# schmidtjonathan/Climate2Weather

Measured on AMD Instinct MI355X. Metric: UNet denoise steps/sec (train fwd+bwd+allreduce+AdamW+EMA windows/s), higher is better.
Workload: dtype bf16; 1 GPU; configs/sda_unet.yml default net, 5 vars x window 13 = 65 ch, 128x128, bf16 training step, 128 windows/GPU/step; global_batch=128, parallelism=dp1, params=72132929

## Files before the change

climate2weather_amd/csrc/conv_igemm.hip:

```cpp
#include <cstdlib>

#include "conv_epilogue.h"
#include "knobs.h"
#include "launch.h"

namespace {

constexpr int BN = 128;
constexpr int WBYTES = BN * 128;
constexpr int NSLOT = 3;
template <int NW> struct GCfg {
    static constexpr int BM = 64 * NW;
    static constexpr int NTHREADS = 128 * NW;
    static constexpr int PBYTES = BM * 128;
    static constexpr int ROWS_PER_ROUND = NTHREADS / 8;
    static constexpr int WROUNDS = BN / ROWS_PER_ROUND;
    static constexpr int ROUND_BYTES = NTHREADS * 16;
};

template <typename T> struct Mma;
template <> struct Mma<bf16_t> {
    __device__ static __forceinline__ void run(const u32x4_t& a, const u32x4_t& b, f32x4_t& c) { c = mfma16<bf16_t>(a, b, c); }
};
template <> struct Mma<f16_t> {
// ... 209 lines not shown
            int ih, iw;
            if (!src_pixel<MODE>(p, oh, ow, tap / 3, tap % 3, ih, iw)) continue;
            const T* xp = (const T*)p.x + (((size_t)b * p.Hin + ih) * p.Win + iw) * p.Cin;
            const T* wp = (const T*)p.w + ((size_t)co * NT + tap) * p.Cin;
            if (co >= p.wrows) continue;
            for (int ci = 0; ci < p.Cin; ++ci) acc = fmaf(Elem<T>::ld(wp + ci), Elem<T>::ld(xp + ci), acc);
        }
        if (p.bias && co < p.wrows) acc += p.bias[co];
        if (p.act == C2W_ACT_SILU) acc = silu_f(acc);
        if (p.act == C2W_ACT_RELU) acc = relu_f(acc);
        const size_t off = (size_t)Q * p.ldy + co;
        if (p.mul) {
            float g = Elem<T>::ld((const T*)p.mul + off);
            acc *= (p.mulmode == C2W_MUL_DSILU) ? dsilu_f(g) : g;
        }
        if (p.res) acc += Elem<T>::ld((const T*)p.res + off);
        if (p.act == C2W_ACT_SILU_PAIR && p.y2) {
            Elem<T>::st((T*)p.y + off, acc);
            const float a_ = Elem<T>::ld((const T*)p.y + off);
            Elem<T>::st((T*)p.y + off, silu_f(a_));
            Elem<T>::st((T*)p.y2 + off, dsilu_f(a_));
            continue;
        }
        if (p.act == C2W_ACT_RELU_PAIR && p.y2) {
            Elem<T>::st((T*)p.y + off, acc);
            const float a_ = Elem<T>::ld((const T*)p.y + off);
            Elem<T>::st((T*)p.y + off, relu_f(a_));
            Elem<T>::st((T*)p.y2 + off, a_ > 0.f ? 1.f : 0.f);
            continue;
        }
        Elem<T>::st((T*)p.y + off, acc);
        if (p.y2) Elem<T>::st((T*)p.y2 + off, silu_f(Elem<T>::ld((const T*)p.y + off)));
    }
}

template <typename T, int MODE, int NW>
int launch_tile(const C2wConvArgs& a, long long npix, int nN, hipStream_t st) {
    typedef GCfg<NW> CF;
    constexpr int ESZ = sizeof(T);
    constexpr int lds_loop = NSLOT * (CF::PBYTES + WBYTES), lds_epi = CF::BM * (BN * ESZ + 16);
    constexpr int lds = lds_loop > lds_epi ? lds_loop : lds_epi;
    if (int rc = c2w_lds_optin<conv_igemm_kernel<T, MODE, NW>>(lds)) return rc;
    const int nM = (int)((npix + CF::BM - 1) / CF::BM);
    conv_igemm_kernel<T, MODE, NW><<<nM * nN, CF::NTHREADS, lds, st>>>(a);
    return (int)hipGetLastError();
}

template <typename T, int MODE>
int launch_mode(const C2wConvArgs& a, int naive, hipStream_t st) {
    const long long npix = (long long)a.B * a.Hout * a.Wout;
    if (naive) {
        long long total = npix * a.Cout;
        int grid = (int)((total + 255) / 256 < 65536 ? (total + 255) / 256 : 65536);
        conv_naive_kernel<T, MODE><<<grid, 256, 0, st>>>(a);
        return (int)hipGetLastError();
    }
    const int nN = (a.Cout + BN - 1) / BN;
    const bool small = ((npix + 255) / 256) * nN < c2w_cu_count();
    return small ? launch_tile<T, MODE, 2>(a, npix, nN, st) : launch_tile<T, MODE, 4>(a, npix, nN, st);
}

template <typename T>
int launch_dtype(const C2wConvArgs& a, int naive, hipStream_t st) {
    switch (a.mode) {
        case C2W_CONV_1X1: return launch_mode<T, C2W_CONV_1X1>(a, naive, st);
        case C2W_CONV_S1: return launch_mode<T, C2W_CONV_S1>(a, naive, st);
        case C2W_CONV_S2: return launch_mode<T, C2W_CONV_S2>(a, naive, st);
        case C2W_CONV_UP: return launch_mode<T, C2W_CONV_UP>(a, naive, st);
        case C2W_CONV_TS2: return launch_mode<T, C2W_CONV_TS2>(a, naive, st);
    }
    return C2W_ERR_BAD_ARG;
}

}

namespace {
C2wKnobs read_knobs() {
    C2wKnobs k;
    k.force_gather = getenv("C2W_FORCE_GATHER") != nullptr;
    k.conv_t3 = getenv("C2W_CONV_T3") ? atoi(getenv("C2W_CONV_T3")) : -1;
    k.conv_s2_patch = getenv("C2W_CONV_S2_PATCH") ? atoi(getenv("C2W_CONV_S2_PATCH")) : 0;
    k.ts2_pairs = !(getenv("C2W_TS2_PAIRS") && atoi(getenv("C2W_TS2_PAIRS")) == 0);
    k.wgrad_atomics = getenv("C2W_WGRAD_ATOMICS") != nullptr;
    k.loss_fusion = getenv("C2W_NO_LOSS_FUSION") == nullptr;
    k.half8 = getenv("C2W_NO_HALF8") == nullptr;
    k.half8_db = !(getenv("C2W_HALF8_DB") && atoi(getenv("C2W_HALF8_DB")) == 0);
    k.attn_valu = getenv("C2W_ATTN_VALU") != nullptr;
    return k;
}
C2wKnobs g_knobs = read_knobs();
}
const C2wKnobs& c2w_knobs() { return g_knobs; }
extern "C" void c2w_knobs_reload(void) { g_knobs = read_knobs(); }

extern "C" int c2w_conv_patch_supported(const C2wConvArgs* a, int dtype) {
    (void)dtype;
    return a != nullptr && c2w_conv_patch_eligible(*a) && !c2w_knobs().force_gather ? 1 : 0;
}

extern "C" int c2w_conv_pool2_supported(const C2wConvArgs* a, int dtype) {
    (void)dtype;
    if (a == nullptr || a->mode != C2W_CONV_S1 || a->res != nullptr || a->mul != nullptr || a->y2 != nullptr || a->act != C2W_ACT_NONE ||
        a->ln_x != nullptr || a->lnf_y != nullptr)
        return 0;
    return c2w_conv_patch_eligible(*a) && !c2w_conv_pair_eligible(*a) && !c2w_knobs().force_gather ? 1 : 0;
}

extern "C" int c2w_conv_lnfwd_supported(const C2wConvArgs* a, int dtype) {
    if (a == nullptr || (dtype != C2W_DTYPE_BF16 && dtype != C2W_DTYPE_F16)) return 0;
    if (a->Cout != 128 || a->ldy != 128 || a->mul != nullptr || a->y2 != nullptr || a->act != C2W_ACT_NONE || a->ln_x != nullptr) return 0;
    return c2w_conv_patch_eligible(*a) && !c2w_knobs().force_gather ? 1 : 0;
}

extern "C" int c2w_conv_lnbwd_supported(const C2wConvArgs* a, int dtype) {
    if (a == nullptr || (dtype != C2W_DTYPE_BF16 && dtype != C2W_DTYPE_F16)) return 0;
    if (a->Cout != 128 || a->ldy != 128 || a->mul != nullptr || a->y2 != nullptr || a->act != C2W_ACT_NONE) return 0;
    return c2w_conv_patch_eligible(*a) && !c2w_knobs().force_gather ? 1 : 0;
}

int c2w_conv_splitk_plan_impl(const C2wConvArgs& a, int dtype, unsigned long long* ws_bytes);
extern "C" int c2w_conv_splitk_plan(const C2wConvArgs* a, int dtype, unsigned long long* ws_bytes) {
    if (a == nullptr) return C2W_ERR_BAD_ARG;
    return c2w_conv_splitk_plan_impl(*a, dtype, ws_bytes);
}

extern "C" int c2w_conv_lnfwd_chain_supported(const C2wConvArgs* a, int dtype) {
    if (!c2w_conv_lnfwd_supported(a, dtype)) return 0;
    return a->mode == C2W_CONV_S1 && c2w_conv_patch3_wanted(*a, dtype) ? 1 : 0;
}

extern "C" int c2w_conv_loss_supported(const C2wConvArgs* a, int dtype) {
    if (a == nullptr || (dtype != C2W_DTYPE_BF16 && dtype != C2W_DTYPE_F16)) return 0;
    if (a->mode != C2W_CONV_S1 || a->wrows > 80 || a->Cout > 128 || a->ldy != 128 || a->res != nullptr || a->mul != nullptr || a->y2 != nullptr ||
        a->act != C2W_ACT_NONE || a->ln_x != nullptr || a->lnf_y != nullptr || (a->flags & C2W_CONV_POOL2) != 0)
        return 0;
    if (a->loss_sum != nullptr && (a->loss_eps == nullptr || a->loss_C <= 0 || a->loss_C != a->wrows || (a->loss_lde & 7) != 0 || a->loss_lde < a->loss_C ||
                                   a->loss_lde > 128))
        return 0;
    const C2wKnobs& k = c2w_knobs();
    return !k.force_gather && k.loss_fusion && c2w_conv_patch_eligible(*a) && c2w_conv_patch3_wanted(*a, dtype) ? 1 : 0;
}

extern "C" long long c2w_conv_det_scratch_bytes(const C2wConvArgs* a, int dtype) {
    if (a == nullptr) return C2W_ERR_BAD_ARG;
    if (a->ln_x != nullptr && a->ln_dm != nullptr) {
        if (!c2w_conv_lnbwd_supported(a, dtype)) return C2W_ERR_UNSUPPORTED;
        return (long long)a->B * (a->Hout >> 3) * (a->Wout >> 4) * 128 * (long long)sizeof(float);
    }
    if (a->loss_sum != nullptr) {
        C2wConvArgs g = *a;
        g.loss_sum = nullptr;
        if (!c2w_conv_loss_supported(&g, dtype)) return C2W_ERR_UNSUPPORTED;
        return (long long)a->B * (a->Hout >> 4) * (a->Wout >> 4) * ((a->Cout + 127) / 128) * (long long)sizeof(float);
    }
    return 0;
}

extern "C" int c2w_conv_wpacked_supported(const C2wConvArgs* a, int dtype) {
    if (a == nullptr || (dtype != C2W_DTYPE_BF16 && dtype != C2W_DTYPE_F16)) return 0;
    return !c2w_knobs().force_gather && c2w_conv_patch_eligible(*a) && c2w_conv_patch3_wanted(*a, dtype) ? 1 : 0;
}

extern "C" int c2w_conv_dispatch(const C2wConvArgs* a, int dtype) {
    if (a == nullptr) return C2W_ERR_BAD_ARG;
    const bool gather = c2w_knobs().force_gather;
    if (!gather && c2w_conv_patch_eligible(*a)) return c2w_conv_patch3_wanted(*a, dtype) ? C2W_KERNEL_PATCH_16X16 : C2W_KERNEL_PATCH_8X16;
    if (!gather && c2w_conv_pair_eligible(*a)) return C2W_KERNEL_PATCH_PAIR;
// ... 47 lines not shown
```

climate2weather_amd/csrc/knobs.h:

```cpp
#pragma once

struct C2wKnobs {
    bool force_gather;
    int conv_t3;
    int conv_s2_patch;
    bool ts2_pairs;
    bool wgrad_atomics;
    bool attn_valu;
    bool loss_fusion;
    bool half8;
    bool half8_db;
};

const C2wKnobs& c2w_knobs();
extern "C" void c2w_knobs_reload(void);
```

climate2weather_amd/csrc/wgrad_patch.hip:

```cpp
#include <algorithm>
#include <cstdint>
#include <cstdlib>
#include <utility>
#include "conv_geom.h"

#include "knobs.h"
#include "launch.h"


namespace {

constexpr int NTHREADS = 512;
constexpr int KPX = 128;
constexpr int ABYTES = KPX * 256;
constexpr int PPITCH = 24;
constexpr int NPIECE = 10 * 3;
constexpr int PBYTES = NPIECE * 1024;
constexpr int NSLOT_A = 3, NSLOT_P = 2;
constexpr int PBASE = NSLOT_A * ABYTES;
constexpr int LDS_BYTES = PBASE + NSLOT_P * PBYTES;

struct WpArgs {
    const void* dy;
    const void* x;
    float* dw;
    float* db;
    int B, H, W, Cin, Cout, ldy;
    int up;
    int ktiles, ktiles_per_split;
    float* ws;
    int direct;
    float* wsb;
    int det;
};

struct WpItem {
    const void* dy;
    const void* x;
    float* dw;
    float* db;
};
constexpr int WP_MAX_ITEMS = 16;
struct WpGroupArgs {
    WpArgs c;
    int n;
    int live_per_item;
    unsigned long long ws_item_floats;
    unsigned long long wsb_item_floats;
    WpItem item[WP_MAX_ITEMS];
};



__device__ __forceinline__ uint32_t sel_oob(bool ok, uint32_t v) {
    asm volatile("" : "+v"(v));
    return ok ? v : C2W_OOB;
}

__device__ __forceinline__ uint32_t swzA(int row) { return (uint32_t)(((row & 3) << 2) | ((row >> 2) & 3)); }
__device__ __forceinline__ uint32_t swzP(int pix) { return (uint32_t)((((pix >> 1) & 1) << 1) | (((pix >> 3) & 1) << 2)); }

__device__ __forceinline__ int wp_xcd_order(int bid, int nblk) {
    const int xcd = bid & 7, q = nblk >> 3, r = nblk & 7;
    return (xcd < r ? xcd * (q + 1) : r * (q + 1) + (xcd - r) * q) + (bid >> 3);
}

template <typename T, bool PAIR = false, bool NARROW = false>
__device__ __forceinline__ void wgrad_patch_body(const WpArgs& p, const int L) {
    constexpr int ESZ = sizeof(T);
    constexpr bool BF = ESZ == 2;
    constexpr int COT = 256 / ESZ;
    constexpr int CIB = 128 / ESZ;
    constexpr int MTW = BF ? 4 : 1;
    extern __shared__ __attribute__((aligned(16))) char smem[];

    const int tid = threadIdx.x, lane = tid & 63;
    const int wid = __builtin_amdgcn_readfirstlane(tid >> 6);
    const int li = lane & 15, lg = lane >> 4;
    static_assert(!NARROW || (BF && !PAIR), "narrow-M form: 16-bit, 16-pixel-wide tiles");
    const int mt0 = BF ? (NARROW ? (wid >> 2) * 4 : (wid & 1) * 4) : (wid >> 1);
    const int nt = BF ? (NARROW ? (wid & 3) : (wid >> 1)) : (wid & 1);
    const bool light = NARROW && wid >= 4;

    const int ncib = p.Cin / CIB;
    const int tilesM = (p.Cout + COT - 1) / COT;
    const int tilesMN = tilesM * ncib;
    const int split = L / tilesMN, mn = L - split * tilesMN;
    const int tm = mn / ncib, cb = mn - tm * ncib;
    const int co0 = tm * COT, ci0 = cb * CIB;
    const int H = p.H, W = p.W;
    const int tw = PAIR ? 1 : W >> 4, tpi = (H >> 3) * tw;
    const int t0 = split * p.ktiles_per_split;
    const int t1 = (t0 + p.ktiles_per_split < p.ktiles) ? t0 + p.ktiles_per_split : p.ktiles;

    const int Ws = p.up ? W >> 1 : W;
    const size_t ximg = (size_t)(p.up ? (H >> 1) * Ws : H * W) * p.Cin * ESZ;
    const size_t yimg = (size_t)H * W * p.ldy * ESZ;
    const uint32_t a_step = PAIR ? (uint32_t)(16 * p.ldy * ESZ) : (uint32_t)(2 * W * p.ldy * ESZ);
    auto dy_voff0 = [&](int tid_) -> uint32_t {
        const int row = tid_ >> 4, pc = tid_ & 15;
        const uint32_t lc = (uint32_t)pc ^ swzA(row);
        const int c = co0 + (int)lc * (16 / ESZ);
        if constexpr (PAIR) {
            return sel_oob(c < p.Cout, (uint32_t)((((row >> 4) * 8 + (row & 7)) * p.ldy + c) * ESZ) + (uint32_t)((row >> 3) & 1) * (uint32_t)yimg);
        } else {
            return sel_oob(c < p.Cout, (uint32_t)((((row >> 4) * W + (row & 15)) * p.ldy + c) * ESZ));
        }
    };
    auto patch_piece = [&](int r) -> int {
        const int pc = r * 8 + wid;
        return pc < NPIECE ? pc : NPIECE - 1;
    };
    auto patch_voff = [&](int r, int lane_, int oh0, int ow0) -> uint32_t {
        const int pc = patch_piece(r);
        const int pr = pc / 3, pg = pc - pr * 3;
        const int px = pg * 8 + (lane_ >> 3);
        const uint32_t lanepart = (uint32_t)(((lane_ & 7) ^ swzP(pr * PPITCH + px)) << 4) + (uint32_t)ci0 * ESZ;
        if constexpr (PAIR) {
            const int pimg = px >= 10 ? 1 : 0;
            const int ih = pr - 1, iw = px - 1 - 10 * pimg;
            const bool ok = (unsigned)ih < 8u && (unsigned)iw < 8u && px < 20;
            return sel_oob(ok, (uint32_t)((ih * 8 + iw) * p.Cin) * ESZ + (uint32_t)pimg * (uint32_t)(64 * p.Cin * ESZ) + lanepart);
        } else {
            const int ih = oh0 - 1 + pr, iw = ow0 - 1 + px;
            const bool ok = (unsigned)ih < (unsigned)H && (unsigned)iw < (unsigned)W && px < 18;
            const int spix = p.up ? (ih >> 1) * Ws + (iw >> 1) : ih * W + iw;
            return sel_oob(ok, (uint32_t)(spix * p.Cin) * ESZ + lanepart);
        }
    };

    auto tile_origin = [&](int t, int& b, int& oh0, int& ow0) {
        b = PAIR ? 2 * t : t / tpi;
        const int tt = PAIR ? 0 : t - (t / tpi) * tpi;
        const int ty = tt / tw, tx = tt - ty * tw;
        b = __builtin_amdgcn_readfirstlane(b);
        oh0 = __builtin_amdgcn_readfirstlane(ty << 3);
        ow0 = __builtin_amdgcn_readfirstlane(tx << 4);
    };
    struct TileSrc {
        __amdgpu_buffer_rsrc_t rsrc;
        int oh0, ow0;
        uint32_t aso;
        char* base;
    };
    auto srcA = [&](int t, int sa) {
        int b, oh0, ow0;
        tile_origin(t, b, oh0, ow0);
        const uint32_t nimg = PAIR && b + 1 < p.B ? 2u : 1u;
        TileSrc s;
        s.rsrc = make_rsrc((const char*)p.dy + (size_t)b * yimg, (uint32_t)yimg * nimg);
        s.oh0 = oh0;
        s.ow0 = ow0;
        s.aso = (uint32_t)((oh0 * W + ow0) * p.ldy) * ESZ;
        s.base = smem + sa * ABYTES + wid * 1024;
        return s;
    };
    auto srcP = [&](int t, int sp) {
        int b, oh0, ow0;
        tile_origin(t, b, oh0, ow0);
        const uint32_t nimg = PAIR && b + 1 < p.B ? 2u : 1u;
        TileSrc s;
        s.rsrc = make_rsrc((const char*)p.x + (size_t)b * ximg, (uint32_t)ximg * nimg);
        s.oh0 = oh0;
        s.ow0 = ow0;
        s.aso = 0;
        s.base = smem + PBASE + sp * PBYTES;
        return s;
    };
    auto pieceA = [&](const TileSrc& s, int i, bool live = true) {
        int tid_ = tid;
        asm volatile("" : "+v"(tid_));
        const uint32_t v = dy_voff0(tid_);
        glds16(s.rsrc, s.base + i * 8192, sel_oob(live, v), s.aso + (uint32_t)i * a_step);
    };
    auto pieceP = [&](const TileSrc& s, int r, bool live = true) {
        int lane_ = lane;
        asm volatile("" : "+v"(lane_));
        const uint32_t v = patch_voff(r, lane_, s.oh0, s.ow0);
        glds16(s.rsrc, s.base + patch_piece(r) * 1024, sel_oob(live, v), 0);
    };
    auto issueA = [&](int t, int sa) {
        const TileSrc s = srcA(t, sa);
#pragma unroll
        for (int i = 0; i < 4; ++i) pieceA(s, i);
    };
    auto issueP = [&](int t, int sp) {
        const TileSrc s = srcP(t, sp);
#pragma unroll
        for (int r = 0; r < 4; ++r) pieceP(s, r);
    };

    f32x4_t acc[9][MTW];
#pragma unroll
    for (int t = 0; t < 9; ++t)
#pragma unroll
        for (int m = 0; m < MTW; ++m) acc[t][m] = (f32x4_t){0.f, 0.f, 0.f, 0.f};
    const bool do_bias = p.db != nullptr && cb == 0 && nt == 0;
    f32x4_t accb[MTW];
#pragma unroll
    for (int m = 0; m < MTW; ++m) accb[m] = (f32x4_t){0.f, 0.f, 0.f, 0.f};

    uint32_t offA[MTW][2], offB[9][2];
    if constexpr (BF) {
        const int qq = li >> 2, pp = li & 3;
#pragma unroll
        for (int h = 0; h < 2; ++h) {
            const int row = 8 * lg + qq + 4 * h;
            const uint32_t f = swzA(row);
#pragma unroll
            for (int m = 0; m < MTW; ++m)
                offA[m][h] = (uint32_t)(row * 256 + (((((mt0 + m) * 2 + (pp >> 1)) ^ f) & 15) << 4) + 8 * (pp & 1));
            const int r = lg >> 1, c = 8 * (lg & 1) + qq + 4 * h;
#pragma unroll
            for (int t = 0; t < 9; ++t) {
                const int pix = (r + t / 3) * PPITCH + c + t % 3 + (PAIR ? 2 * (lg & 1) : 0);
                offB[t][h] = (uint32_t)(pix * 128 + (((uint32_t)(nt * 2 + (pp >> 1)) ^ swzP(pix)) << 4) + 8 * (pp & 1));
            }
        }
    }

    if (t0 < t1) {
        issueP(t0, 0);
        issueA(t0, 0);
        const TileSrc s1 = srcA(t0 + 1 < t1 ? t0 + 1 : t0, 1);
#pragma unroll
        for (int i = 0; i < 4; ++i) pieceA(s1, i, t0 + 1 < t1);
    }
    int sa = 0, sp = 0;
    for (int t = t0; t < t1; ++t) {
        asm volatile("s_waitcnt vmcnt(4)" ::: "memory");
        __builtin_amdgcn_s_barrier();
        const bool hasP = t + 1 < t1, hasA = t + 2 < t1;
        const TileSrc nP = srcP(hasP ? t + 1 : t, sp ^ 1), nA = srcA(hasA ? t + 2 : t, sa == 0 ? 2 : sa - 1);
        if constexpr (!BF) {
#pragma unroll
            for (int r = 0; r < 4; ++r) pieceP(nP, r, hasP);
#pragma unroll
            for (int i = 0; i < 4; ++i) pieceA(nA, i, hasA);
        }
        const char* const SA = smem + sa * ABYTES;
        const char* const SP = smem + PBASE + sp * PBYTES;
        if constexpr (BF) {
            const uint32_t sA = (uint32_t)(uintptr_t)SA, sP = (uint32_t)(uintptr_t)SP;
            auto rd = [&](tr_frag& f, uint32_t base, uint32_t o0, uint32_t o1, auto IMMc) {
                constexpr int IMM = decltype(IMMc)::value;
                asm volatile("ds_read_b64_tr_b16 %0, %1 offset:%2" : "=v"(f.lo) : "v"(base + o0), "n"(IMM));
                asm volatile("ds_read_b64_tr_b16 %0, %1 offset:%2" : "=v"(f.hi) : "v"(base + o1), "n"(IMM));
            };
            static_for<4>([&](auto KSc) {
                constexpr int ks = decltype(KSc)::value;
                {
                    const bool first = wid < 4;
                    if ((ks == 0 && first) || (ks == 1 && !first)) {
#pragma unroll
                        for (int r = 0; r < 4; ++r) pieceP(nP, r, hasP);
                    }
                    if ((ks == 2 && first) || (ks == 3 && !first)) {
#pragma unroll
                        for (int i = 0; i < 4; ++i) pieceA(nA, i, hasA);
                    }
                }
                constexpr int PF = 2;
                tr_frag a[MTW], bq[PF + 1];
                rd(a[0], sA, offA[0][0], offA[0][1], IC<ks * 32 * 256>{});
                if (!light) {
#pragma unroll
                    for (int m = 1; m < MTW; ++m) rd(a[m], sA, offA[m][0], offA[m][1], IC<ks * 32 * 256>{});
                }
                static_for<PF>([&](auto Jc) {
                    constexpr int j = decltype(Jc)::value;
                    rd(bq[j], sP, offB[j][0], offB[j][1], IC<ks * 2 * PPITCH * 128>{});
                });
                static_for<9>([&](auto TPc) {
                    constexpr int tp = decltype(TPc)::value;
                    if constexpr (tp + PF < 9) rd(bq[(tp + PF) % (PF + 1)], sP, offB[tp + PF][0], offB[tp + PF][1], IC<ks * 2 * PPITCH * 128>{});
                    constexpr int AHEAD = (tp + PF < 9 ? PF : 8 - tp) * 2;
                    if constexpr (AHEAD == 4) asm volatile("s_waitcnt lgkmcnt(4)" ::: "memory");
                    else if constexpr (AHEAD == 2) asm volatile("s_waitcnt lgkmcnt(2)" ::: "memory");
                    else asm volatile("s_waitcnt lgkmcnt(0)" ::: "memory");
                    __builtin_amdgcn_sched_barrier(0);
                    const bf16x8_t bfr = bq[tp % (PF + 1)].vec();
                    acc[tp][0] = mfma16s<T>(a[0].vec(), bfr, acc[tp][0]);
                    if (!light) {
#pragma unroll
                        for (int m = 1; m < MTW; ++m) acc[tp][m] = mfma16s<T>(a[m].vec(), bfr, acc[tp][m]);
                    }
                    if (tp == 8 && do_bias) {
                        const bf16x8_t ones = __builtin_bit_cast(bf16x8_t, ones16<T>());
                        accb[0] = mfma16s<T>(a[0].vec(), ones, accb[0]);
                        if (!light) {
#pragma unroll
                            for (int m = 1; m < MTW; ++m) accb[m] = mfma16s<T>(a[m].vec(), ones, accb[m]);
                        }
                    }
                    __builtin_amdgcn_sched_barrier(0);
                });
            });
        } else {
#pragma unroll 4
            for (int kk = 0; kk < 32; ++kk) {
                const int row = kk * 4 + lg;
                const float a = *(const float*)(SA + row * 256 + ((((uint32_t)(mt0 * 4 + (li >> 2))) ^ swzA(row)) << 4) + (li & 3) * 4);
                const int r = kk >> 2, c = 4 * (kk & 3) + lg;
#pragma unroll
                for (int tp = 0; tp < 9; ++tp) {
                    const int pix = (r + tp / 3) * PPITCH + c + tp % 3 + (PAIR && (kk & 2) ? 2 : 0);
                    const float bv = *(const float*)(SP + pix * 128 + ((((uint32_t)(nt * 4 + (li >> 2))) ^ swzP(pix)) << 4) + (li & 3) * 4);
                    acc[tp][0] = __builtin_amdgcn_mfma_f32_16x16x4f32(a, bv, acc[tp][0], 0, 0, 0);
                }
                if (do_bias) accb[0] = __builtin_amdgcn_mfma_f32_16x16x4f32(a, 1.0f, accb[0], 0, 0, 0);
            }
        }
        sa = sa == 2 ? 0 : sa + 1;
        sp ^= 1;
    }

    if (t0 >= t1) return;
    if (do_bias && li == 0) {
#pragma unroll
        for (int m = 0; m < MTW; ++m)
#pragma unroll
            for (int r = 0; r < 4; ++r) {
                const int row = (mt0 + m) * 16 + lg * 4 + r;
                const int co = co0 + row;
                if (p.det) {
                    if (p.wsb != nullptr) p.wsb[((size_t)split * tilesM + tm) * COT + row] = accb[m][r];
                    else if (co < p.Cout) p.db[co] = p.db[co] + accb[m][r];
                } else if (co < p.Cout) {
                    atomicAdd(p.db + co, accb[m][r]);
                }
            }
    }
    constexpr int OS = CIB + 4;
    float* const O = (float*)smem;
#pragma unroll
    for (int tp = 0; tp < 9; ++tp) {
        __syncthreads();
#pragma unroll
        for (int m = 0; m < MTW; ++m)
#pragma unroll
            for (int r = 0; r < 4; ++r) O[((mt0 + m) * 16 + lg * 4 + r) * OS + nt * 16 + li] = acc[tp][m][r];
        __syncthreads();
        if (p.ws != nullptr) {
            float* const dst = p.ws + (((size_t)split * tilesMN + mn) * 9 + tp) * (COT * CIB);
            for (int idx = tid; idx < COT * CIB; idx += NTHREADS) dst[idx] = O[(idx / CIB) * OS + (idx % CIB)];
        } else if (p.direct) {
            for (int idx = tid; idx < COT * CIB; idx += NTHREADS) {
                const int row = idx / CIB, col = idx - row * CIB;
                const int co = co0 + row;
                if (co < p.Cout) {
                    float* const d = p.dw + ((size_t)co * 9 + tp) * p.Cin + ci0 + col;
                    *d = *d + O[row * OS + col];
                }
            }
        } else {
            for (int idx = tid; idx < COT * CIB; idx += NTHREADS) {
                const int row = idx / CIB, col = idx - row * CIB;
                const int co = co0 + row;
                if (co < p.Cout) atomicAdd(p.dw + ((size_t)co * 9 + tp) * p.Cin + ci0 + col, O[row * OS + col]);
            }
        }
    }
}

template <typename T, bool PAIR = false, bool NARROW = false>
__global__ __launch_bounds__(NTHREADS, 2) void wgrad_patch_kernel(const WpArgs p) {
    wgrad_patch_body<T, PAIR, NARROW>(p, wp_xcd_order((int)blockIdx.x, (int)gridDim.x));
}

typedef __attribute__((address_space(4))) const char wp_kernarg_t;
__device__ __forceinline__ WpItem wp_item(int it) {
    const WpItem __attribute__((address_space(4)))* tab =
        (const WpItem __attribute__((address_space(4)))*)((wp_kernarg_t*)__builtin_amdgcn_kernarg_segment_ptr() + offsetof(WpGroupArgs, item));
    WpItem r;
    r.dy = tab[it].dy;
    r.x = tab[it].x;
    r.dw = tab[it].dw;
    r.db = tab[it].db;
    return r;
}

template <typename T, bool PAIR = false>
__global__ __launch_bounds__(NTHREADS, 2) void wgrad_patch_group_kernel(const WpGroupArgs g) {
    const int Lg = wp_xcd_order((int)blockIdx.x, (int)gridDim.x);
    const int it = __builtin_amdgcn_readfirstlane(Lg / g.live_per_item);
    const int L = Lg - it * g.live_per_item;
    const WpItem e = wp_item(it);
    WpArgs p = g.c;
    p.dy = e.dy;
    p.x = e.x;
    p.dw = e.dw;
    p.db = e.db;
    p.ws = g.c.ws != nullptr ? g.c.ws + (size_t)it * g.ws_item_floats : nullptr;
    p.wsb = g.c.wsb != nullptr ? g.c.wsb + (size_t)it * g.wsb_item_floats : nullptr;
    wgrad_patch_body<T, PAIR, false>(p, L);
}

struct WgradBiasReduce {
    const float* wsb;
    float* db;
    int cols, tpo, nmain;
};
static inline WgradBiasReduce bias_reduce_of(const float* wsb, float* db, int cols, int nsplit, int nmain) {
    WgradBiasReduce br;
    br.wsb = wsb; br.db = db; br.cols = cols; br.tpo = det_reduce_tpo(nsplit); br.nmain = nmain;
    return br;
}

#ifndef C2W_RED_COLS
#define C2W_RED_COLS 64
#endif
template <int COT, int CIB>
__device__ __forceinline__ void wgrad_reduce_body(const float* __restrict__ ws, float* __restrict__ dw, int nsplit, int tilesMN, int ncib,
                                                  int Cin, int Cout, int nblk) {
    constexpr int RC = C2W_RED_COLS, RG = 256 / RC;
    __shared__ f32x4_t red[RG][RC];
    const size_t per4 = (size_t)tilesMN * 9 * COT * CIB / 4;
    const f32x4_t* ws4 = (const f32x4_t*)ws;
    const int q = threadIdx.x % RC, grp = threadIdx.x / RC;
    for (size_t base = (size_t)blockIdx.x * RC; base < per4; base += (size_t)nblk * RC) {
        const size_t i4 = base + q;
        f32x4_t acc = {0.f, 0.f, 0.f, 0.f};
        if (i4 < per4) {
#pragma unroll 8
            for (int sidx = grp; sidx < nsplit; sidx += RG) acc += ws4[(size_t)sidx * per4 + i4];
        }
        red[grp][q] = acc;
        __syncthreads();
        if (grp == 0 && i4 < per4) {
#pragma unroll
            for (int g2 = 1; g2 < RG; ++g2) acc += red[g2][q];
            const size_t i = i4 * 4;
            const int col = (int)(i % CIB);
            size_t r = i / CIB;
            const int row = (int)(r % COT);
            r /= COT;
            const int tp = (int)(r % 9);
            const int mn = (int)(r / 9);
            const int tm = mn / ncib, cb = mn - tm * ncib;
            const int co = tm * COT + row;
            if (co < Cout) {
                f32x4_t* d = (f32x4_t*)(dw + ((size_t)co * 9 + tp) * Cin + cb * CIB + col);
                *d = *d + acc;
            }
        }
        __syncthreads();
    }
}

template <int COT, int CIB>
__global__ __launch_bounds__(256) void wgrad_reduce_kernel(const float* __restrict__ ws, float* __restrict__ dw, int nsplit, int tilesMN, int ncib,
                                                           int Cin, int Cout, WgradBiasReduce br) {
    if ((int)blockIdx.x >= br.nmain) {
        det_reduce_body(br.wsb, br.db, nsplit, Cout, Cout, 0, br.tpo, br.cols, (int)blockIdx.x - br.nmain);
        return;
    }
    wgrad_reduce_body<COT, CIB>(ws, dw, nsplit, tilesMN, ncib, Cin, Cout, br.nmain);
}
template <int COT, int CIB>
__global__ __launch_bounds__(256) void wgrad_reduce_group_kernel(const WpGroupArgs g, int nsplit, int tilesMN, int ncib, WgradBiasReduce br) {
    const int it = (int)blockIdx.y;
    const WpItem e = wp_item(it);
    if ((int)blockIdx.x >= br.nmain) {
        if (e.db != nullptr)
            det_reduce_body(g.c.wsb + (size_t)it * g.wsb_item_floats, e.db, nsplit, g.c.Cout, g.c.Cout, 0, br.tpo, br.cols, (int)blockIdx.x - br.nmain);
        return;
    }
    wgrad_reduce_body<COT, CIB>(g.c.ws + (size_t)it * g.ws_item_floats, e.dw, nsplit, tilesMN, ncib, g.c.Cin, g.c.Cout, br.nmain);
}

template <int ESZ, bool PAIR>
static void split_plan(const C2wConvArgs& a, int& ktiles, int& tilesMN, int& nsplit, int& ktiles_per_split) {
    constexpr int COT = 256 / ESZ, CIB = 128 / ESZ;
    ktiles = PAIR ? ((a.B + 1) >> 1) * (a.Hout >> 3) : a.B * (a.Hout >> 3) * (a.Wout >> 4);
    tilesMN = ((a.Cout + COT - 1) / COT) * (a.Cin / CIB);
    nsplit = c2w_cu_count() / tilesMN;
    if (nsplit > ktiles) nsplit = ktiles;
    if (nsplit < 1) nsplit = 1;
    ktiles_per_split = (ktiles + nsplit - 1) / nsplit;
    nsplit = (ktiles + ktiles_per_split - 1) / ktiles_per_split;
}

template <int ESZ, bool PAIR>
static size_t ws_need(const C2wConvArgs& a) {
    constexpr int COT = 256 / ESZ, CIB = 128 / ESZ;
    int ktiles, tilesMN, nsplit, per;
    split_plan<ESZ, PAIR>(a, ktiles, tilesMN, nsplit, per);
    const size_t bias_rows = (a.flags & C2W_CONV_DETERMINISTIC) ? (size_t)nsplit * ((a.Cout + COT - 1) / COT) * COT * sizeof(float) : 0;
    return nsplit > 1 ? (size_t)nsplit * tilesMN * 9 * COT * CIB * sizeof(float) + bias_rows : 0;
}

template <typename T, bool PAIR, bool NARROW = false>
int launch(const C2wConvArgs& a, float* dw, float* db, float* ws, size_t ws_bytes, hipStream_t st) {
    constexpr int ESZ = sizeof(T);
    constexpr int COT = 256 / ESZ, CIB = 128 / ESZ;
    WpArgs p;
    p.dy = a.y; p.x = a.x; p.dw = dw; p.db = db;
    p.B = a.B; p.H = a.Hout; p.W = a.Wout; p.Cin = a.Cin; p.Cout = a.Cout; p.ldy = a.ldy;
    p.up = a.mode == C2W_CONV_UP ? 1 : 0;
    int tilesMN, nsplit;
    split_plan<ESZ, PAIR>(a, p.ktiles, tilesMN, nsplit, p.ktiles_per_split);
    if (int rc = c2w_lds_optin<wgrad_patch_kernel<T, PAIR, NARROW>>(LDS_BYTES)) return rc;
    const size_t need = (size_t)nsplit * tilesMN * 9 * COT * CIB * sizeof(float);
    const int bias_cols = (tilesMN / (a.Cin / CIB)) * COT;
    p.det = (a.flags & C2W_CONV_DETERMINISTIC) ? 1 : 0;
    if (p.det) {
        if (c2w_knobs().wgrad_atomics) return C2W_ERR_BAD_ARG;
        if (nsplit > 1 && (ws == nullptr || need + (size_t)nsplit * bias_cols * sizeof(float) > ws_bytes)) return C2W_ERR_BAD_ARG;
    }
    p.ws = (ws != nullptr && need <= ws_bytes && nsplit > 1 && !c2w_knobs().wgrad_atomics) ? ws : nullptr;
    p.wsb = p.det && nsplit > 1 && db != nullptr ? ws + need / sizeof(float) : nullptr;
    p.direct = nsplit == 1 && !c2w_knobs().wgrad_atomics ? 1 : 0;
    wgrad_patch_kernel<T, PAIR, NARROW><<<tilesMN * nsplit, NTHREADS, LDS_BYTES, st>>>(p);
    if (p.ws != nullptr) {
        const size_t per_split = (size_t)tilesMN * 9 * COT * CIB;
        const int grid = (int)std::min<size_t>((per_split / 4 + C2W_RED_COLS - 1) / C2W_RED_COLS, 8192);
        const int extra = p.wsb != nullptr ? det_reduce_blocks(nsplit, a.Cout) : 0;
        wgrad_reduce_kernel<COT, CIB><<<grid + extra, 256, 0, st>>>(p.ws, dw, nsplit, tilesMN, a.Cin / CIB, a.Cin, a.Cout,
                                                                    bias_reduce_of(p.wsb, db, bias_cols, nsplit, grid));
    }
    return (int)hipGetLastError();
}

static void group_plan(int n, int tilesMN, int ktiles, int& nsplit, int& ktiles_per_split) {
    const int T = n * tilesMN, cus = c2w_cu_count();
    double best = 1e30;
    nsplit = 1;
    for (int r = 0; r <= 4; ++r) {
        int ns = r == 0 ? 1 : (cus * r) / T;
        if (ns < 1) ns = 1;
        if (ns > ktiles) ns = ktiles;
        const int per = (ktiles + ns - 1) / ns;
        ns = (ktiles + per - 1) / per;
        const int rounds = (T * ns + cus - 1) / cus;
        const double cost = rounds * (per * 4.1 + (ns > 1 ? 28.0 : 16.0)) + (ns > 1 ? 10.0 : 0.0);
        if (cost < best - 1e-9) {
            best = cost;
            nsplit = ns;
        }
    }
    ktiles_per_split = (ktiles + nsplit - 1) / nsplit;
}

template <int ESZ, bool PAIR>
static size_t group_ws_need(const C2wConvArgs& a, int n) {
    constexpr int COT = 256 / ESZ, CIB = 128 / ESZ;
    int ktiles, tilesMN, ns1, per1, nsplit, per;
    split_plan<ESZ, PAIR>(a, ktiles, tilesMN, ns1, per1);
    group_plan(n, tilesMN, ktiles, nsplit, per);
    const size_t bias_rows = (a.flags & C2W_CONV_DETERMINISTIC) ? (size_t)n * nsplit * ((a.Cout + COT - 1) / COT) * COT * sizeof(float) : 0;
    return nsplit > 1 ? (size_t)n * nsplit * tilesMN * 9 * COT * CIB * sizeof(float) + bias_rows : 0;
}

template <typename T, bool PAIR>
int launch_group(const C2wConvArgs& a, const C2wWgradItem* items, int n, float* ws, size_t ws_bytes, hipStream_t st) {
    constexpr int ESZ = sizeof(T);
    constexpr int COT = 256 / ESZ, CIB = 128 / ESZ;
    WpGroupArgs g;
    WpArgs& p = g.c;
    p.dy = nullptr; p.x = nullptr; p.dw = nullptr; p.db = nullptr;
    p.B = a.B; p.H = a.Hout; p.W = a.Wout; p.Cin = a.Cin; p.Cout = a.Cout; p.ldy = a.ldy;
    p.up = a.mode == C2W_CONV_UP ? 1 : 0;
    int tilesMN, ns1, per1, nsplit;
    split_plan<ESZ, PAIR>(a, p.ktiles, tilesMN, ns1, per1);
    group_plan(n, tilesMN, p.ktiles, nsplit, p.ktiles_per_split);
    const size_t item_floats = (size_t)nsplit * tilesMN * 9 * COT * CIB;
    const int bias_cols = (tilesMN / (a.Cin / CIB)) * COT;
    p.det = (a.flags & C2W_CONV_DETERMINISTIC) ? 1 : 0;
    const size_t bias_item_floats = p.det ? (size_t)nsplit * bias_cols : 0;
    if (nsplit > 1 && (ws == nullptr || (size_t)n * (item_floats + bias_item_floats) * sizeof(float) > ws_bytes)) return C2W_ERR_BAD_ARG;
    p.ws = nsplit > 1 ? ws : nullptr;
    p.wsb = p.det && nsplit > 1 ? ws + (size_t)n * item_floats : nullptr;
    g.wsb_item_floats = bias_item_floats;
    p.direct = nsplit == 1 ? 1 : 0;
    g.n = n;
    g.live_per_item = tilesMN * nsplit;
    g.ws_item_floats = item_floats;
    for (int i = 0; i < WP_MAX_ITEMS; ++i) {
        const C2wWgradItem& e = items[i < n ? i : n - 1];
        g.item[i].dy = e.dy; g.item[i].x = e.x; g.item[i].dw = e.dw; g.item[i].db = e.dbias;
    }
    if (int rc = c2w_lds_optin<wgrad_patch_group_kernel<T, PAIR>>(LDS_BYTES)) return rc;
    wgrad_patch_group_kernel<T, PAIR><<<g.live_per_item * n, NTHREADS, LDS_BYTES, st>>>(g);
    if (p.ws != nullptr) {
        const size_t per_split = (size_t)tilesMN * 9 * COT * CIB;
        const int grid = (int)std::min<size_t>((per_split / 4 + C2W_RED_COLS - 1) / C2W_RED_COLS, 8192);
        const int extra = p.wsb != nullptr ? det_reduce_blocks(nsplit, a.Cout) : 0;
        wgrad_reduce_group_kernel<COT, CIB><<<dim3(grid + extra, n), 256, 0, st>>>(g, nsplit, tilesMN, a.Cin / CIB,
                                                                                   bias_reduce_of(p.wsb, nullptr, bias_cols, nsplit, grid));
    }
    return (int)hipGetLastError();
}

}

bool c2w_wgrad_patch_group_eligible(const C2wConvArgs& a, int n, int dtype) {
    const bool narrow = dtype != C2W_DTYPE_F32 && !c2w_wgrad_patch_pair(a) && a.Cout <= 80;
    return c2w_wgrad_patch_eligible(a) && n >= 2 && n <= WP_MAX_ITEMS && !narrow && !c2w_knobs().wgrad_atomics;
}

int c2w_wgrad_patch_group(const C2wConvArgs& a, const C2wWgradItem* items, int n, float* ws, size_t ws_bytes, int dtype, hipStream_t st) {
    if (c2w_wgrad_patch_pair(a)) return c2w_by_dtype(dtype, [&](auto t) { return launch_group<decltype(t), true>(a, items, n, ws, ws_bytes, st); });
    return c2w_by_dtype(dtype, [&](auto t) { return launch_group<decltype(t), false>(a, items, n, ws, ws_bytes, st); });
}

size_t c2w_wgrad_patch_group_ws_bytes(const C2wConvArgs& a, int n, int dtype) {
    const bool pair = c2w_wgrad_patch_pair(a);
    if (dtype == C2W_DTYPE_F32) return pair ? group_ws_need<4, true>(a, n) : group_ws_need<4, false>(a, n);
    return pair ? group_ws_need<2, true>(a, n) : group_ws_need<2, false>(a, n);
}

bool c2w_wgrad_patch_pair(const C2wConvArgs& a) {
    return a.mode == C2W_CONV_S1 && a.Win == 8 && a.Hin == 8;
}

bool c2w_wgrad_patch_eligible(const C2wConvArgs& a) {
    if (a.mode == C2W_CONV_UP)
        return a.Hout == 2 * a.Hin && a.Wout == 2 * a.Win && (a.Hout & 7) == 0 && (a.Wout & 15) == 0;
    return a.mode == C2W_CONV_S1 && a.Hin == a.Hout && a.Win == a.Wout && (a.Hin & 7) == 0 && ((a.Win & 15) == 0 || c2w_wgrad_patch_pair(a));
}

int c2w_wgrad_patch(const C2wConvArgs& a, float* dw, float* db, float* ws, size_t ws_bytes, int dtype, hipStream_t st) {
    if (c2w_wgrad_patch_pair(a)) return c2w_by_dtype(dtype, [&](auto t) { return launch<decltype(t), true>(a, dw, db, ws, ws_bytes, st); });
    if (dtype != C2W_DTYPE_F32 && a.Cout <= 80)
        return c2w_by_dtype16(dtype, [&](auto t) { return launch<decltype(t), false, true>(a, dw, db, ws, ws_bytes, st); });
    return c2w_by_dtype(dtype, [&](auto t) { return launch<decltype(t), false>(a, dw, db, ws, ws_bytes, st); });
}

size_t c2w_wgrad_patch_ws_bytes(const C2wConvArgs& a, int dtype) {
    const bool pair = c2w_wgrad_patch_pair(a);
    if (dtype == C2W_DTYPE_F32) return pair ? ws_need<4, true>(a) : ws_need<4, false>(a);
    return pair ? ws_need<2, true>(a) : ws_need<2, false>(a);
}
```

Before: 2781 windows/s.

## Compute upsample-conv weight grads on source grid with folded 2x2 taps

Adds a source-grid variant of the patch-based weight-gradient kernel for nearest-upsample convolutions. Each output-row parity class is handled by its own split. The 3x3 taps collapse onto a 2x2 footprint of the low-resolution input, so each k-step issues 4 MFMA fragments instead of 9, and the results are folded back into 9 taps in the epilogue. This removes redundant multiplies on duplicated upsampled pixels. In exchange it doubles the number of workspace splits and the reduction traffic, and adds index-mapping complexity. It is enabled by default for bf16/fp16 upsample layers with Cout > 80 when the workspace is large enough.

Measured after the change: 2805 windows/s (median of 6 runs). No clear change (+0.9%).

```diff
diff --git a/climate2weather_amd/csrc/conv_igemm.hip b/climate2weather_amd/csrc/conv_igemm.hip
--- a/climate2weather_amd/csrc/conv_igemm.hip
+++ b/climate2weather_amd/csrc/conv_igemm.hip
@@ -315,7 +315,8 @@
     k.conv_s2_patch = getenv("C2W_CONV_S2_PATCH") ? atoi(getenv("C2W_CONV_S2_PATCH")) : 0;
     k.ts2_pairs = !(getenv("C2W_TS2_PAIRS") && atoi(getenv("C2W_TS2_PAIRS")) == 0);
     k.wgrad_atomics = getenv("C2W_WGRAD_ATOMICS") != nullptr;
-    k.loss_fusion = getenv("C2W_NO_LOSS_FUSION") == nullptr;
+    k.wgrad_up_source = !(getenv("C2W_WGRAD_UP_SOURCE") && atoi(getenv("C2W_WGRAD_UP_SOURCE")) == 0);
+    k.loss_fusion =getenv("C2W_NO_LOSS_FUSION") == nullptr;
     k.half8 = getenv("C2W_NO_HALF8") == nullptr;
     k.half8_db = !(getenv("C2W_HALF8_DB") && atoi(getenv("C2W_HALF8_DB")) == 0);
     k.attn_valu = getenv("C2W_ATTN_VALU") != nullptr;
diff --git a/climate2weather_amd/csrc/knobs.h b/climate2weather_amd/csrc/knobs.h
--- a/climate2weather_amd/csrc/knobs.h
+++ b/climate2weather_amd/csrc/knobs.h
@@ -6,6 +6,7 @@
     int conv_s2_patch;
     bool ts2_pairs;
     bool wgrad_atomics;
+    bool wgrad_up_source;
     bool attn_valu;
     bool loss_fusion;
     bool half8;
diff --git a/climate2weather_amd/csrc/wgrad_patch.hip b/climate2weather_amd/csrc/wgrad_patch.hip
--- a/climate2weather_amd/csrc/wgrad_patch.hip
+++ b/climate2weather_amd/csrc/wgrad_patch.hip
@@ -6,6 +6,7 @@
 
 #include "knobs.h"
 #include "launch.h"
+#include "wgrad_upsrc_maps.h"
 
 
 namespace {
@@ -65,7 +66,7 @@
     return (xcd < r ? xcd * (q + 1) : r * (q + 1) + (xcd - r) * q) + (bid >> 3);
 }
 
-template <typename T, bool PAIR = false, bool NARROW = false>
+template <typename T, bool PAIR = false, bool NARROW = false, bool UPSRC = false>
 __device__ __forceinline__ void wgrad_patch_body(const WpArgs& p, const int L) {
     constexpr int ESZ = sizeof(T);
     constexpr bool BF = ESZ == 2;
@@ -78,6 +79,8 @@
     const int wid = __builtin_amdgcn_readfirstlane(tid >> 6);
     const int li = lane & 15, lg = lane >> 4;
     static_assert(!NARROW || (BF && !PAIR), "narrow-M form: 16-bit, 16-pixel-wide tiles");
+    static_assert(!UPSRC || (BF && !PAIR && !NARROW), "source-grid form: 16-bit, 16-pixel-wide tiles, full co tiles");
+    constexpr int NFRAG = UPSRC ? 4 : 9;
     const int mt0 = BF ? (NARROW ? (wid >> 2) * 4 : (wid & 1) * 4) : (wid >> 1);
     const int nt = BF ? (NARROW ? (wid & 3) : (wid >> 1)) : (wid & 1);
     const bool light = NARROW && wid >= 4;
@@ -89,19 +92,22 @@
     const int tm = mn / ncib, cb = mn - tm * ncib;
     const int co0 = tm * COT, ci0 = cb * CIB;
     const int H = p.H, W = p.W;
-    const int tw = PAIR ? 1 : W >> 4, tpi = (H >> 3) * tw;
-    const int t0 = split * p.ktiles_per_split;
+    const int tw = PAIR ? 1 : W >> 4, tpi = (H >> (UPSRC ? 4 : 3)) * tw;
+    const int cls = UPSRC ? upsrc::cls_of(split) : 0;
+    const int t0 = (UPSRC ? upsrc::ksplit_of(split) : split) * p.ktiles_per_split;
     const int t1 = (t0 + p.ktiles_per_split < p.ktiles) ? t0 + p.ktiles_per_split : p.ktiles;
 
     const int Ws = p.up ? W >> 1 : W;
     const size_t ximg = (size_t)(p.up ? (H >> 1) * Ws : H * W) * p.Cin * ESZ;
     const size_t yimg = (size_t)H * W * p.ldy * ESZ;
-    const uint32_t a_step = PAIR ? (uint32_t)(16 * p.ldy * ESZ) : (uint32_t)(2 * W * p.ldy * ESZ);
+    const uint32_t a_step = PAIR ? (uint32_t)(16 * p.ldy * ESZ) : (uint32_t)((UPSRC ? 4 : 2) * W * p.ldy * ESZ);
     auto dy_voff0 = [&](int tid_) -> uint32_t {
         const int row = tid_ >> 4, pc = tid_ & 15;
-        const uint32_t lc = (uint32_t)pc ^ swzA(row);
+        const uint32_t lc = (uint32_t)pc ^ (UPSRC ? upsrc::swz_dy(row) : swzA(row));
         const int c = co0 + (int)lc * (16 / ESZ);
-        if constexpr (PAIR) {
+        if constexpr (UPSRC) {
+            return sel_oob(c < p.Cout, (uint32_t)((((row >> 4) * 2 * W + (row & 15)) * p.ldy + c) * ESZ));
+        } else if constexpr (PAIR) {
             return sel_oob(c < p.Cout, (uint32_t)((((row >> 4) * 8 + (row & 7)) * p.ldy + c) * ESZ) + (uint32_t)((row >> 3) & 1) * (uint32_t)yimg);
         } else {
             return sel_oob(c < p.Cout, (uint32_t)((((row >> 4) * W + (row & 15)) * p.ldy + c) * ESZ));
@@ -109,10 +115,18 @@
     };
     auto patch_piece = [&](int r) -> int {
         const int pc = r * 8 + wid;
-        return pc < NPIECE ? pc : NPIECE - 1;
+        constexpr int NP = UPSRC ? upsrc::NPIECE : NPIECE;
+        return pc < NP ? pc : NP - 1;
     };
     auto patch_voff = [&](int r, int lane_, int oh0, int ow0) -> uint32_t {
         const int pc = patch_piece(r);
+        if constexpr (UPSRC) {
+            const int pr = pc >> 1, px = (pc & 1) * 8 + (lane_ >> 3);
+            const uint32_t lanepart = (uint32_t)(((lane_ & 7) ^ upsrc::swz_patch(pr * upsrc::PITCH + px)) << 4) + (uint32_t)ci0 * ESZ;
+            const int ih = upsrc::patch_ih(oh0, cls, pr), iw = upsrc::patch_iw(ow0, px);
+            const bool ok = (unsigned)ih < (unsigned)(H >> 1) && (unsigned)iw < (unsigned)Ws && px < upsrc::COLS;
+            return sel_oob(ok, (uint32_t)((ih * Ws + iw) * p.Cin) * ESZ + lanepart);
+        }
         const int pr = pc / 3, pg = pc - pr * 3;
         const int px = pg * 8 + (lane_ >> 3);
         const uint32_t lanepart = (uint32_t)(((lane_ & 7) ^ swzP(pr * PPITCH + px)) << 4) + (uint32_t)ci0 * ESZ;
@@ -134,7 +148,7 @@
         const int tt = PAIR ? 0 : t - (t / tpi) * tpi;
         const int ty = tt / tw, tx = tt - ty * tw;
         b = __builtin_amdgcn_readfirstlane(b);
-        oh0 = __builtin_amdgcn_readfirstlane(ty << 3);
+        oh0 = __builtin_amdgcn_readfirstlane(ty << (UPSRC ? 4 : 3));
         ow0 = __builtin_amdgcn_readfirstlane(tx << 4);
     };
     struct TileSrc {
@@ -151,7 +165,7 @@
         s.rsrc = make_rsrc((const char*)p.dy + (size_t)b * yimg, (uint32_t)yimg * nimg);
         s.oh0 = oh0;
         s.ow0 = ow0;
-        s.aso = (uint32_t)((oh0 * W + ow0) * p.ldy) * ESZ;
+        s.aso = (uint32_t)(((oh0 + cls) * W + ow0) * p.ldy) * ESZ;
         s.base = smem + sa * ABYTES + wid * 1024;
         return s;
     };
@@ -205,16 +219,21 @@
         const int qq = li >> 2, pp = li & 3;
 #pragma unroll
         for (int h = 0; h < 2; ++h) {
-            const int row = 8 * lg + qq + 4 * h;
-            const uint32_t f = swzA(row);
+            const int row = UPSRC ? 16 * lg + 8 * h + 2 * qq : 8 * lg + qq + 4 * h;
+            const uint32_t f = UPSRC ? upsrc::swz_dy(row) : swzA(row);
 #pragma unroll
             for (int m = 0; m < MTW; ++m)
                 offA[m][h] = (uint32_t)(row * 256 + (((((mt0 + m) * 2 + (pp >> 1)) ^ f) & 15) << 4) + 8 * (pp & 1));
             const int r = lg >> 1, c = 8 * (lg & 1) + qq + 4 * h;
 #pragma unroll
             for (int t = 0; t < 9; ++t) {
-                const int pix = (r + t / 3) * PPITCH + c + t % 3 + (PAIR ? 2 * (lg & 1) : 0);
-                offB[t][h] = (uint32_t)(pix * 128 + (((uint32_t)(nt * 2 + (pp >> 1)) ^ swzP(pix)) << 4) + 8 * (pp & 1));
+                if constexpr (UPSRC) {
+                    const int pix = (lg + t / 3) * upsrc::PITCH + 4 * h + qq + t % 3;
+                    offB[t][h] = (uint32_t)(pix * 128 + (((uint32_t)(nt * 2 + (pp >> 1)) ^ upsrc::swz_patch(pix)) << 4) + 8 * (pp & 1));
+                } else {
+                    const int pix = (r + t / 3) * PPITCH + c + t % 3 + (PAIR ? 2 * (lg & 1) : 0);
+                    offB[t][h] = (uint32_t)(pix * 128 + (((uint32_t)(nt * 2 + (pp >> 1)) ^ swzP(pix)) << 4) + 8 * (pp & 1));
+                }
             }
         }
     }
@@ -262,30 +281,40 @@
                 }
                 constexpr int PF = 2;
                 tr_frag a[MTW], bq[PF + 1];
-                rd(a[0], sA, offA[0][0], offA[0][1], IC<ks * 32 * 256>{});
+                constexpr int IMMA = UPSRC ? (ks >> 1) * 64 * 256 + (ks & 1) * 256 : ks * 32 * 256;
+                constexpr int IMMB = UPSRC ? (ks >> 1) * 4 * upsrc::PITCH * 128 : ks * 2 * PPITCH * 128;
+                auto bsel = [](auto FRc) {
+                    constexpr int fr = decltype(FRc)::value;
+                    return IC<UPSRC ? 3 * (fr >> 1) + (ks & 1) + (fr & 1) : fr>{};
+                };
+                rd(a[0], sA, offA[0][0], offA[0][1], IC<IMMA>{});
                 if (!light) {
 #pragma unroll
-                    for (int m = 1; m < MTW; ++m) rd(a[m], sA, offA[m][0], offA[m][1], IC<ks * 32 * 256>{});
+                    for (int m = 1; m < MTW; ++m) rd(a[m], sA, offA[m][0], offA[m][1], IC<IMMA>{});
                 }
                 static_for<PF>([&](auto Jc) {
-                    constexpr int j = decltype(Jc)::value;
-                    rd(bq[j], sP, offB[j][0], offB[j][1], IC<ks * 2 * PPITCH * 128>{});
+                    constexpr int j = decltype(bsel(Jc))::value;
+                    rd(bq[decltype(Jc)::value], sP, offB[j][0], offB[j][1], IC<IMMB>{});
                 });
-                static_for<9>([&](auto TPc) {
-                    constexpr int tp = decltype(TPc)::value;
-                    if constexpr (tp + PF < 9) rd(bq[(tp + PF) % (PF + 1)], sP, offB[tp + PF][0], offB[tp + PF][1], IC<ks * 2 * PPITCH * 128>{});
-                    constexpr int AHEAD = (tp + PF < 9 ? PF : 8 - tp) * 2;
+                static_for<NFRAG>([&](auto TPc) {
+                    constexpr int fr = decltype(TPc)::value;
+                    constexpr int tp = UPSRC ? upsrc::g_index(fr >> 1, ks & 1, fr & 1) : fr;
+                    if constexpr (fr + PF < NFRAG) {
+                        constexpr int j = decltype(bsel(IC<fr + PF>{}))::value;
+                        rd(bq[(fr + PF) % (PF + 1)], sP, offB[j][0], offB[j][1], IC<IMMB>{});
+                    }
+                    constexpr int AHEAD = (fr + PF < NFRAG ? PF : NFRAG - 1 - fr) * 2;
                     if constexpr (AHEAD == 4) asm volatile("s_waitcnt lgkmcnt(4)" ::: "memory");
                     else if constexpr (AHEAD == 2) asm volatile("s_waitcnt lgkmcnt(2)" ::: "memory");
                     else asm volatile("s_waitcnt lgkmcnt(0)" ::: "memory");
                     __builtin_amdgcn_sched_barrier(0);
-                    const bf16x8_t bfr = bq[tp % (PF + 1)].vec();
+                    const bf16x8_t bfr = bq[fr % (PF + 1)].vec();
                     acc[tp][0] = mfma16s<T>(a[0].vec(), bfr, acc[tp][0]);
                     if (!light) {
 #pragma unroll
                         for (int m = 1; m < MTW; ++m) acc[tp][m] = mfma16s<T>(a[m].vec(), bfr, acc[tp][m]);
                     }
-                    if (tp == 8 && do_bias) {
+                    if (fr == NFRAG - 1 && do_bias) {
                         const bf16x8_t ones = __builtin_bit_cast(bf16x8_t, ones16<T>());
                         accb[0] = mfma16s<T>(a[0].vec(), ones, accb[0]);
                         if (!light) {
@@ -339,7 +368,19 @@
 #pragma unroll
         for (int m = 0; m < MTW; ++m)
 #pragma unroll
-            for (int r = 0; r < 4; ++r) O[((mt0 + m) * 16 + lg * 4 + r) * OS + nt * 16 + li] = acc[tp][m][r];
+            for (int r = 0; r < 4; ++r) {
+                float v;
+                if constexpr (UPSRC) {
+                    const int c0 = upsrc::fold_c(0, tp % 3), c1 = upsrc::fold_c(1, tp % 3);
+                    const int r0 = upsrc::fold_r(0, tp / 3), r1 = upsrc::fold_r(1, tp / 3);
+                    const float v0 = acc[upsrc::g_index(r0, 0, c0)][m][r] + acc[upsrc::g_index(r0, 1, c1)][m][r];
+                    const float v1 = acc[upsrc::g_index(r1, 0, c0)][m][r] + acc[upsrc::g_index(r1, 1, c1)][m][r];
+                    v = cls ? v1 : v0;
+                } else {
+                    v = acc[tp][m][r];
+                }
+                O[((mt0 + m) * 16 + lg * 4 + r) * OS + nt * 16 + li] = v;
+            }
         __syncthreads();
         if (p.ws != nullptr) {
             float* const dst = p.ws + (((size_t)split * tilesMN + mn) * 9 + tp) * (COT * CIB);
@@ -363,9 +404,9 @@
     }
 }
 
-template <typename T, bool PAIR = false, bool NARROW = false>
+template <typename T, bool PAIR = false, bool NARROW = false, bool UPSRC = false>
 __global__ __launch_bounds__(NTHREADS, 2) void wgrad_patch_kernel(const WpArgs p) {
-    wgrad_patch_body<T, PAIR, NARROW>(p, wp_xcd_order((int)blockIdx.x, (int)gridDim.x));
+    wgrad_patch_body<T, PAIR, NARROW, UPSRC>(p, wp_xcd_order((int)blockIdx.x, (int)gridDim.x));
 }
 
 typedef __attribute__((address_space(4))) const char wp_kernarg_t;
@@ -481,13 +522,63 @@
     nsplit = (ktiles + ktiles_per_split - 1) / ktiles_per_split;
 }
 
+static bool upsrc_geometry(const C2wConvArgs& a, int dtype) {
+    if (a.mode != C2W_CONV_UP || dtype == C2W_DTYPE_F32 || (a.Hout & 15) != 0 || (a.Wout & 15) != 0 || a.Cout <= 80) return false;
+    int ktiles, tilesMN, nsplit, per;
+    split_plan<2, false>(a, ktiles, tilesMN, nsplit, per);
+    return nsplit > 1;
+}
+static void upsrc_plan(const C2wConvArgs& a, int& ktiles, int& tilesMN, int& nsplit, int& ktiles_per_split) {
+    ktiles = a.B * (a.Hout >> 4) * (a.Wout >> 4);
+    tilesMN = ((a.Cout + 127) / 128) * (a.Cin / 64);
+    nsplit = c2w_cu_count() / (2 * tilesMN);
+    if (nsplit > ktiles) nsplit = ktiles;
+    if (nsplit < 1) nsplit = 1;
+    ktiles_per_split = (ktiles + nsplit - 1) / nsplit;
+    nsplit = (ktiles + ktiles_per_split - 1) / ktiles_per_split;
+}
+static size_t upsrc_ws_need(const C2wConvArgs& a) {
+    int ktiles, tilesMN, nsplit, per;
+    upsrc_plan(a, ktiles, tilesMN, nsplit, per);
+    const size_t bias_rows = (a.flags & C2W_CONV_DETERMINISTIC) ? (size_t)2 * nsplit * ((a.Cout + 127) / 128) * 128 * sizeof(float) : 0;
+    return (size_t)2 * nsplit * tilesMN * 9 * 128 * 64 * sizeof(float) + bias_rows;
+}
+
 template <int ESZ, bool PAIR>
 static size_t ws_need(const C2wConvArgs& a) {
     constexpr int COT = 256 / ESZ, CIB = 128 / ESZ;
     int ktiles, tilesMN, nsplit, per;
     split_plan<ESZ, PAIR>(a, ktiles, tilesMN, nsplit, per);
     const size_t bias_rows = (a.flags & C2W_CONV_DETERMINISTIC) ? (size_t)nsplit * ((a.Cout + COT - 1) / COT) * COT * sizeof(float) : 0;
-    return nsplit > 1 ? (size_t)nsplit * tilesMN * 9 * COT * CIB * sizeof(float) + bias_rows : 0;
+    const size_t need = nsplit > 1 ? (size_t)nsplit * tilesMN * 9 * COT * CIB * sizeof(float) + bias_rows : 0;
+    if (ESZ == 2 && !PAIR && upsrc_geometry(a, C2W_DTYPE_BF16)) return std::max(need, upsrc_ws_need(a));
+    return need;
+}
+
+template <typename T>
+int launch_upsrc(const C2wConvArgs& a, float* dw, float* db, float* ws, hipStream_t st) {
+    constexpr int COT = 128, CIB = 64;
+    WpArgs p;
+    p.dy = a.y; p.x = a.x; p.dw = dw; p.db = db;
+    p.B = a.B; p.H = a.Hout; p.W = a.Wout; p.Cin = a.Cin; p.Cout = a.Cout; p.ldy = a.ldy;
+    p.up = 1;
+    int tilesMN, nsplit;
+    upsrc_plan(a, p.ktiles, tilesMN, nsplit, p.ktiles_per_split);
+    if (int rc = c2w_lds_optin<wgrad_patch_kernel<T, false, false, true>>(LDS_BYTES)) return rc;
+    const int nws = 2 * nsplit;
+    const size_t need = (size_t)nws * tilesMN * 9 * COT * CIB * sizeof(float);
+    const int bias_cols = (tilesMN / (a.Cin / CIB)) * COT;
+    p.det = (a.flags & C2W_CONV_DETERMINISTIC) ? 1 : 0;
+    p.ws = ws;
+    p.wsb = p.det && db != nullptr ? ws + need / sizeof(float) : nullptr;
+    p.direct = 0;
+    wgrad_patch_kernel<T, false, false, true><<<tilesMN * nws, NTHREADS, LDS_BYTES, st>>>(p);
+    const size_t per_split = (size_t)tilesMN * 9 * COT * CIB;
+    const int grid = (int)std::min<size_t>((per_split / 4 + C2W_RED_COLS - 1) / C2W_RED_COLS, 8192);
+    const int extra = p.wsb != nullptr ? det_reduce_blocks(nws, a.Cout) : 0;
+    wgrad_reduce_kernel<COT, CIB><<<grid + extra, 256, 0, st>>>(p.ws, dw, nws, tilesMN, a.Cin / CIB, a.Cin, a.Cout,
+                                                                bias_reduce_of(p.wsb, db, bias_cols, nws, grid));
+    return (int)hipGetLastError();
 }
 
 template <typename T, bool PAIR, bool NARROW = false>
@@ -622,6 +713,8 @@
 
 int c2w_wgrad_patch(const C2wConvArgs& a, float* dw, float* db, float* ws, size_t ws_bytes, int dtype, hipStream_t st) {
     if (c2w_wgrad_patch_pair(a)) return c2w_by_dtype(dtype, [&](auto t) { return launch<decltype(t), true>(a, dw, db, ws, ws_bytes, st); });
+    if (upsrc_geometry(a, dtype) && c2w_knobs().wgrad_up_source && !c2w_knobs().wgrad_atomics && ws != nullptr && upsrc_ws_need(a) <= ws_bytes)
+        return c2w_by_dtype16(dtype, [&](auto t) { return launch_upsrc<decltype(t)>(a, dw, db, ws, st); });
     if (dtype != C2W_DTYPE_F32 && a.Cout <= 80)
         return c2w_by_dtype16(dtype, [&](auto t) { return launch<decltype(t), false, true>(a, dw, db, ws, ws_bytes, st); });
     return c2w_by_dtype(dtype, [&](auto t) { return launch<decltype(t), false>(a, dw, db, ws, ws_bytes, st); });
diff --git a/climate2weather_amd/csrc/wgrad_upsrc_maps.h b/climate2weather_amd/csrc/wgrad_upsrc_maps.h
--- /dev/null
+++ b/climate2weather_amd/csrc/wgrad_upsrc_maps.h
@@ -0,0 +1,45 @@
+#ifndef C2W_WGRAD_UPSRC_MAPS_H
+#define C2W_WGRAD_UPSRC_MAPS_H
+
+#include "core_side.h"
+
+namespace upsrc {
+
+constexpr int ROWS = 9, COLS = 10;
+constexpr int PITCH = 16;
+constexpr int NPIECE = ROWS * 2;
+constexpr int NG = 8;
+
+C2W_BOTH constexpr int ws_split(int L, int tilesMN) { return L / tilesMN; }
+C2W_BOTH constexpr int cls_of(int wsplit) { return wsplit & 1; }
+C2W_BOTH constexpr int ksplit_of(int wsplit) { return wsplit >> 1; }
+
+C2W_BOTH constexpr int tiles_per_image(int H, int W) { return (H >> 4) * (W >> 4); }
+C2W_BOTH constexpr int tile_oh0(int tt, int W) { return (tt / (W >> 4)) << 4; }
+C2W_BOTH constexpr int tile_ow0(int tt, int W) { return (tt % (W >> 4)) << 4; }
+C2W_BOTH constexpr int tile_oh(int oh0, int a, int q) { return oh0 + 2 * (q >> 4) + a; }
+C2W_BOTH constexpr int tile_ow(int ow0, int q) { return ow0 + (q & 15); }
+
+C2W_BOTH constexpr int patch_ih(int oh0, int a, int pr) { return (oh0 >> 1) - 1 + a + pr; }
+C2W_BOTH constexpr int patch_iw(int ow0, int pc) { return (ow0 >> 1) - 1 + pc; }
+
+C2W_BOTH constexpr int step_b(int ks) { return ks & 1; }
+C2W_BOTH constexpr int step_half(int ks) { return ks >> 1; }
+C2W_BOTH constexpr int step_i(int ks, int kk) { return 4 * step_half(ks) + (kk >> 3); }
+C2W_BOTH constexpr int step_j(int kk) { return kk & 7; }
+C2W_BOTH constexpr int step_pixel(int ks, int kk) { return 16 * step_i(ks, kk) + 2 * step_j(kk) + step_b(ks); }
+C2W_BOTH constexpr int step_patch_row(int ks, int kk, int ri) { return step_i(ks, kk) + ri; }
+C2W_BOTH constexpr int step_patch_col(int ks, int kk, int ci) { return step_j(kk) + step_b(ks) + ci; }
+
+C2W_BOTH constexpr int rho(int a, int dy) { return a == 0 ? (dy == 0 ? -1 : 0) : (dy == 2 ? 1 : 0); }
+C2W_BOTH constexpr int gamma(int b, int dx) { return rho(b, dx); }
+C2W_BOTH constexpr int fold_r(int a, int dy) { return rho(a, dy) + 1 - a; }
+C2W_BOTH constexpr int fold_c(int b, int dx) { return gamma(b, dx) + 1 - b; }
+C2W_BOTH constexpr int g_index(int ri, int b, int ci) { return (ri * 2 + b) * 2 + ci; }
+
+C2W_BOTH constexpr unsigned swz_dy(int q) { return (unsigned)((((q >> 1) & 3) << 2) | (((q >> 4) & 1) << 1) | ((q >> 3) & 1)); }
+C2W_BOTH constexpr unsigned swz_patch(int pix) { return (unsigned)((((pix >> 1) & 1) << 1) | (((pix >> 4) & 1) << 2)); }
+
+}
+
+#endif
```
